# degleris1/CMF.jl

Measured on AMD Instinct MI355X. Metric: MU iters/sec (convolutive NMF multiplicative update; achieved HBM GB/s in `hbm`), higher is better.
Workload: dtype f32

## Files before the change

### cmf.jl_amd/csrc/cmf_api.hip

```cpp
#include "cmf_internal.h"

static void wb_free(cmf_handle_s *h);
static void wb_disarm(cmf_handle_s *h);

size_t n_partial(const cmf_handle_s *h)
{
    const CmfDims &d = h->d;
    size_t n = (size_t)(64 * h->conv_gx) * (size_t)std::max(h->conv_gy, h->conv_gy_ext);
    n = std::max(n, (size_t)(d.Np / 64) * d.KB * d.L);
    n = std::max(n, (size_t)((d.Tl + 63) / 64) * d.KB);
    n = std::max(n, 2 * (((size_t)d.Tl * d.K32 + 1023) / 1024));
    return n;
}

static int ensure_stage(cmf_handle_s *h, size_t elems)
{
    if (h->stage_elems >= elems) return CMF_OK;
    if (h->stage) HIPCHK(hipFree(h->stage));
    h->stage = nullptr;
    h->stage_elems = 0;
    HIPCHK(hipMalloc(&h->stage, elems * sizeof(double)));
    h->stage_elems = elems;
    return CMF_OK;
}
// ... 328 lines not shown
        for (const Want &w : wants) {
            *w.pp = static_cast<char *>(h->arena) + off;
            off += (w.bytes + 255) & ~(size_t)255;
        }
        h->numden = h->numden_own;
        for (int w = 0; w < 4; ++w) h->halo[w] = h->halo_own[w];
        h->d_scalar = h->d_scalar_own;
    }
    HIPB(hipHostMalloc(&h->h_scalar, 4 * sizeof(double)));
    if (data) {
        TRYB(upload_cols(h, data, 0, Tl, true, true));
        if (h->halo_r > 0) TRYB(upload_cols(h, data + (size_t)Tl * N, Tl, h->halo_r, false, false));
        h->data_norm = std::sqrt(h->data_sumsq);
        h->have_data = true;
    }
#undef TRYB
#undef HIPB
    *out = h;
    return CMF_OK;
}


int launch_hxt_on(cmf_handle_s *h, const float *X0, const float *X1, int NpX, int nsrc, float *slabs, int nchunks, int chunk_len,
                         int main_rows)
{
    ProfScope prof_(h, hxt_prof_class(h, X0, nsrc));
    const CmfDims &d = h->d;
    h->spec_gen = -1;
    HxtParams p;
    p.H = h->H; p.X0 = X0; p.X1 = X1; p.slabs = slabs;
    p.Np = NpX; p.K32 = d.K32; p.KB = d.KB; p.PADL = d.PADL; p.L = d.L; p.Tl = main_rows >= 0 ? main_rows : d.Tl; p.chunk_len = chunk_len;
    p.G = h->hxt_groups; p.nsrc = nsrc;
    p.CG = hxt_cg(nchunks);
    dim3 grid((NpX / 128) * p.CG * h->hxt_groups, nchunks / p.CG, nsrc * d.KB), block(256);
    switch (h->hxt_LP) {
#define CASE(LP_) case LP_: hipLaunchKernelGGL((hxt_kernel<LP_>), grid, block, 0, h->stream, p); break;
        CASE(1) CASE(2) CASE(3) CASE(4) CASE(5) CASE(6) CASE(8)
#undef CASE
    default: return fail(CMF_ERR_STATE, "internal: bad hxt LP %d", h->hxt_LP);
    }
    for (int i = 0; i < 7; ++i)
        if (kHxtLP[i] == h->hxt_LP) h->launches[LA_HXT + i] += 1;
    h->launches[nsrc == 1 ? LA_HXT_NSRC1 : LA_HXT_NSRC2] += 1;
    h->launches[p.Tl < d.Tl ? LA_HXT_TAIL : LA_HXT_NO_TAIL] += 1;
    KCHK("hxt_kernel");
    return CMF_OK;
}

int launch_transconv(cmf_handle_s *h, int nsrc, const float *xt0, bool front_block)
{
    if (h->sk_tc) return launch_transconv_small(h, nsrc, xt0);
    ProfScope prof_(h, nsrc == 2 ? PROF_TRANSCONV : PROF_TRANSCONV_1);
    const CmfDims &d = h->d;
    TcParams p;
    p.Wn = h->Wn; p.XT0 = xt0 ? xt0 : h->XT; p.XT1 = h->estT; p.slabs = h->hslabs;
    p.NpW = d.Np;
    p.TP = d.TP; p.PADL = d.PADL; p.K32 = d.K32; p.KB = d.KB; p.L = d.L; p.Tl = d.Tl;
    p.nsrc = nsrc;
    p.C = (int)(rup(d.N, 8) / 8);
    p.W = nsrc == 2 ? h->tc_W : h->tc_W1;
    p.F = nsrc == 2 ? h->tc_S : h->tc_S1;
    p.wtab = h->tc_tab[nsrc == 2 ? 0 : 1];
    p.t_first = 0;
    p.slab_rows = d.Tl;
    if (front_block) {
        p.W = h->tc_W2; p.F = h->tc_S2; p.wtab = h->tc_tab[2];
        p.t_first = -128;
        p.slab_rows = d.Tl + 128;
// ... 8 lines not shown
    h->launches[LA_TC + h->tc_LT / 4 - 1] += 1;
    if (front_block) h->launches[LA_TC_FRONT] += 1;
    if (p.W >= 64 && p.W % 32 == 0) h->launches[LA_TC_XCD] += 1;
    KCHK("transconv_kernel");
    return CMF_OK;
}

int launch_slab_sum(cmf_handle_s *h, float *out, const float *in, int nslabs, size_t stride, bool take_carry,
                           CmfHxtTail tail)
{
    size_t n4 = stride / 4;
    int blocks = (int)std::min<size_t>(2048, (n4 + 255) / 256);
    CmfLossCarry carry{};
    if (take_carry && h->carry.partial) {
        carry = h->carry;
        h->carry = CmfLossCarry{};
    }
    hipLaunchKernelGGL(slab_sum_kernel, dim3(blocks + (carry.partial ? 1 : 0)), dim3(256), 0, h->stream, out, in, nslabs, stride, n4, carry, tail);
    h->launches[carry.partial ? LA_SLAB_SUM_CARRY : LA_SLAB_SUM] += 1;
    KCHK("slab_sum_kernel");
    return CMF_OK;
}

int hxt_contract(cmf_handle_s *h, const float *X0, const float *X1, int nsrc, float *out, bool take_carry, bool slabs_only)
{
    const CmfDims &d = h->d;
    h->spec_gen = -1;
    if (h->small_k) return hxt_contract_small(h, X0, X1, nsrc, out, take_carry, slabs_only);
    const int nch = nsrc == 2 ? h->hxt_nchunks : h->hxt_nchunks1, clen = nsrc == 2 ? h->hxt_chunk_len : h->hxt_chunk_len1;
    const int main_rows = nsrc == 2 ? h->hxt_main : h->hxt_main1;
    CMFTRY(launch_hxt_on(h, X0, X1, d.Np, nsrc, h->wslabs, nch, clen, main_rows));
    const CmfHxtTail tail{h->H, X0, X1, d.Tl - main_rows, d.PADL + main_rows, d.L, d.K32, d.Np};
    return launch_slab_sum(h, out, h->wslabs, hxt_nslabs(nch), (size_t)nsrc * d.L * d.K32 * d.Np, take_carry, tail);
}

int read_scalar(cmf_handle_s *h, int slot, double *v)
{
    HIPCHK(hipMemcpyAsync(h->h_scalar + slot, h->d_scalar + slot, sizeof(double), hipMemcpyDeviceToHost, h->stream));
    HIPCHK(hipStreamSynchronize(h->stream));
    *v = h->h_scalar[slot];
    return CMF_OK;
}

static int check_ready(cmf_handle_s *h, bool need_data)
{
    if (!h) return fail(CMF_ERR_ARG, "handle is NULL");
    if (h->root_only) return fail(CMF_ERR_STATE, "this entry needs a single-GPU handle, not the front handle of a cmf_create_multi group");
    HIPCHK(hipSetDevice(h->device));
    if (!h->factors_set) return fail(CMF_ERR_STATE, "factors not set: call cmf_set_factors first");
    if (need_data && !h->have_data) return fail(CMF_ERR_STATE, "handle was created without data");
    return CMF_OK;
}

// ... 19 lines not shown
    default: return fail(CMF_ERR_STATE, "internal: the MU rule launches no conv mode %d", conv_mode(family, base));
    }
}

static int mu_conv(cmf_handle_s *h, int base, float *out, int T_store, int gy)
{
    const MuForm &f = mu_form(h);
    return mu_launch_conv(h, base >= CONV_BASE_LOSS ? f.loss_family : f.store_family, base, out, T_store, gy, mu_buf(h, f.conv_data[base]));
}

static bool mu_est_current(const cmf_handle_s *h) { return h->reuse_est && h->est_kind == mu_est_kind(h); }

static bool w_speculated(cmf_handle_s *h)
{
    const bool hit = mu_form(h).square_fusions && h->spec_gen >= 0 && h->spec_gen == h->est_gen && mu_est_current(h) && !h->carry.partial;
    h->spec_gen = -1;
    if (hit) h->spec_hits += 1;
    return hit;
}

static int mu_contract_c2(cmf_handle_s *h, bool slabs_only)
{
    const MuForm &f = mu_form(h);
    return hxt_contract(h, mu_buf(h, f.c2_src[0]), mu_buf(h, f.c2_src[1]), f.c2_nsrc, slabs_only ? nullptr : h->numden, !slabs_only, slabs_only);
}

static int mu_contract_w(cmf_handle_s *h, bool slabs_only)
{
    if (w_speculated(h)) return CMF_OK;
    if (!mu_est_current(h)) CMFTRY(mu_conv(h, CONV_BASE_STORE, h->est, h->d.Tl, h->conv_gy));
    set_est(h, mu_est_kind(h));
    return mu_contract_c2(h, slabs_only);
}

int w_partial_impl(cmf_handle_s *h) { return mu_contract_w(h, false); }

int w_partial_half_impl(cmf_handle_s *h, int den)
{
    const CmfDims &d = h->d;
    const size_t LKN = (size_t)d.L * d.K32 * d.Np;
    if (den) {
        if (!(h->reuse_est && h->est_kind == EST_CONV))
            CMFTRY(launch_conv<CONV_EST>(h, h->est, d.Tl, h->conv_gy));
        set_est(h, EST_CONV);
    }
    const float *src = den ? h->est : h->X;
    return hxt_contract(h, src, src, 1, h->numden + (den ? LKN : 0), den != 0);
}

int w_apply_impl(cmf_handle_s *h, double l1W, double l2W, const float *tail_src, float *tail_dst, int tail_n, const float *den)
{
    const CmfDims &d = h->d;
    dim3 grid(d.Np / 64, d.KB, d.L);
    if (!den) den = h->numden + (size_t)d.L * d.K32 * d.Np;
    const bool root = mu_form(h).sqrt_update;
    hipLaunchKernelGGL(root ? w_update_sqrt_kernel : w_update_kernel, grid, dim3(256), 0, h->stream, h->Wt, h->Wn, h->numden, den,
                       d.N, d.K, d.L, d.Np, d.K32, (float)l1W, (float)(2.0 * l2W), tail_src, tail_dst, tail_n);
    KCHK(root ? "w_update_sqrt_kernel" : "w_update_kernel");
    set_est(h, EST_NONE);
    return CMF_OK;
}

static int w_phase_impl(cmf_handle_s *h, double l1W, double l2W)
{
    const CmfDims &d = h->d;
    const MuForm &f = mu_form(h);
    if (!(h->small_k && f.square_fusions)) {
        CMFTRY(w_partial_impl(h));
        if (f.kl_den()) {
            hipLaunchKernelGGL(kl_hsum_kernel, dim3(d.K, KL_HCHUNKS), dim3(256), 0, h->stream, h->Ht, d.TP, d.PADL, d.Tl, h->kl_sums);
            KCHK("kl_hsum_kernel");
            hipLaunchKernelGGL(kl_den_w_kernel, dim3(d.L, d.K), dim3(256), 0, h->stream, h->Ht, h->kl_sums, h->numden + (size_t)d.L * d.K32 * d.Np, d.TP, d.PADL, d.Tl,
                               d.K32, d.Np);
            KCHK("kl_den_w_kernel");
        }
        return w_apply_impl(h, l1W, l2W);
    }
    CMFTRY(mu_contract_w(h, true));
    CmfLossCarry carry{};
    if (h->carry.partial) {
// ... 510 lines not shown
{
    if (!h) return fail(CMF_ERR_ARG, "handle is NULL");
    if (h->group) return group_sync(h->group);
    HIPCHK(hipSetDevice(h->device));
    HIPCHK(hipStreamSynchronize(h->stream));
    return CMF_OK;
}

int cmf_rccl_version(int *version, char *path, int64_t path_len)
{
    if (!version) return fail(CMF_ERR_ARG, "version is NULL");
    CMFTRY(rccl_load());
    RCCLCHK(g_rccl.GetVersion(version));
    if (path && path_len > 0) snprintf(path, (size_t)path_len, "%s", g_rccl.path.c_str());
    return CMF_OK;
}

int cmf_get_counter(cmf_handle h, const char *name, int64_t *value)
{
    if (!h || !name || !value) return fail(CMF_ERR_ARG, "NULL argument");
    if (std::strcmp(name, "hals_pipeline_reruns") == 0) { *value = h->hals_reruns; return CMF_OK; }
    if (std::strcmp(name, "writeback_calls") == 0) { *value = h->wb ? h->wb->armed_calls : 0; return CMF_OK; }
    if (std::strcmp(name, "speculated_contractions") == 0) { *value = h->spec_hits; return CMF_OK; }
    if (std::strcmp(name, "liveness_checks") == 0) { *value = g_liveness_checks.load(); return CMF_OK; }
    if (admm_counter(h, name, value)) return CMF_OK;
    if (sep_counter(h, name, value)) return CMF_OK;
    if (anls_counter(h, name, value)) return CMF_OK;
    if (std::strcmp(name, "small_k_fused_h_updates") == 0) {
        *value = h->sk_fused_h;
        if (h->group)
            for (const cmf_handle_s *s : h->group->sh) *value += (s != h) ? s->sk_fused_h : 0;
        return CMF_OK;
    }
    if (std::strcmp(name, "writeback_overlapped") == 0) { *value = h->wb ? h->wb->hooked_calls : 0; return CMF_OK; }
    if (std::strncmp(name, "launches:", 9) == 0) {
        for (int c = 0; c < LA_NCLS; ++c)
            if (std::strcmp(name + 9, kLaunchNames[c]) == 0) {
                *value = h->launches[c];
                if (h->group)
                    for (const cmf_handle_s *s : h->group->sh) *value += (s != h) ? s->launches[c] : 0;
                return CMF_OK;
            }
        return fail(CMF_ERR_ARG, "unknown launch path '%s'", name + 9);
    }
    if (h->group) {
        cmf_group_s *g = h->group;
// ... 39 lines not shown
    return CMF_OK;
}

int cmf_set_option(cmf_handle h, const char *name, int value)
{
    if (!h || !name) return fail(CMF_ERR_ARG, "NULL argument");
    if (std::strcmp(name, "anls_backup_only") == 0) {
        if (h->group || h->root_only || h->sharded) return fail(CMF_ERR_UNSUPPORTED, "anls_backup_only: the ANLS rule runs on single-GPU handles only");
        if (value != 0 && value != 1) return fail(CMF_ERR_ARG, "anls_backup_only must be 0 or 1");
        h->anls_backup_only = value;
        return CMF_OK;
    }
    if (std::strcmp(name, "nnls_large") == 0) {
        if (h->group || h->root_only || h->sharded) return fail(CMF_ERR_UNSUPPORTED, "nnls_large: the ANLS rule and the separable fit run on single-GPU handles only");
        if (value != 0 && value != 1) return fail(CMF_ERR_ARG, "nnls_large must be 0 or 1");
        h->nnls_large = value;
        return CMF_OK;
    }
    if (std::strcmp(name, "kl_mask") == 0) {
        if (h->group || h->root_only || h->sharded) return fail(CMF_ERR_UNSUPPORTED, "kl_mask: the mask and the divergence of the MU rule are chosen on single-GPU handles only");
        if (value != 0 && value != 1) return fail(CMF_ERR_ARG, "kl_mask must be 0 or 1");
        if (!value && h->mu_mask && h->mu_div) return fail(CMF_ERR_STATE, "kl_mask: the KL form and a mask are both installed; clear the mask or restore CMF_DIV_SQUARE first");
        h->kl_mask = value;
        return CMF_OK;
    }
    if (std::strcmp(name, "is_div") == 0) {
        if (h->group || h->root_only || h->sharded) return fail(CMF_ERR_UNSUPPORTED, "is_div: the divergence of the MU rule is chosen on single-GPU handles only");
        if (value != 0 && value != 1) return fail(CMF_ERR_ARG, "is_div must be 0 or 1");
        if (!value && h->mu_div == CMF_DIV_IS) return fail(CMF_ERR_STATE, "is_div: the Itakura-Saito divergence is installed; restore CMF_DIV_SQUARE with cmf_mu_set_divergence first");
        h->is_div = value;
        return CMF_OK;
    }
    if (h->group) {
        cmf_group_s *g = h->group;
        CMFTRY(group_join(g));
        if (std::strcmp(name, "allreduce_overlap") == 0) {
            CMFTRY(group_sync(g));
            if (value) CMFTRY(group_ensure_lane1(g));
            g->overlap = value != 0;
            g->num_ready = false;
            return CMF_OK;
        }
        if (std::strcmp(name, "halo_in_allreduce") == 0) {
            CMFTRY(group_sync(g));
            g->halo_opt = value != 0;
            g->halos_current = false;
// ... 1176 lines not shown
```

### cmf.jl_amd/csrc/cmf_internal.h

```cpp
#pragma once
#pragma GCC visibility push(default)
#include "cmf_hip.h"
#pragma GCC visibility pop
#include "cmf_kernels.h"
#include "cmf_rng.h"
#include "cmf_writeback.h"

#include <algorithm>
#include <atomic>
#include <chrono>
#include <cmath>
#include <cstdarg>
#include <cstdio>
#include <cstring>
#include <functional>
#include <map>
#include <mutex>
#include <string>
#include <thread>
#include <vector>

inline thread_local std::string g_err;

static int fail(int code, const char *fmt, ...)
// ... 232 lines not shown
    bool have_data = false;
    bool reuse_est = true;
    int gram = 0;
    float *gram_numden_h = nullptr;
    bool prof = false;
    int prof_every = 1;
    int prof_seen[32] = {0};
    int64_t launches[LA_NCLS] = {0};
    struct ProfRec { hipEvent_t a, b; int cls; };
    unsigned prof_mask = 0;
    std::vector<ProfRec> prof_recs;
    std::vector<hipEvent_t> prof_pool;
    int est_kind = EST_NONE;
    void *arena = nullptr;
    size_t arena_bytes = 0;
    bool streams_may_hang = false;
    int64_t est_gen = 0;
    int64_t spec_gen = -1;
    int last_rule_call = 0;
    bool speculate = true;
    std::function<int()> after_reduce;
    int64_t hals_spec_gen = -1;
    int64_t spec_hits = 0;

    struct cmf_group_s *group = nullptr;
    bool root_only = false;
    hipStream_t own_comm_stream = nullptr, comm_stream = nullptr;
    hipEvent_t ev_c0 = nullptr, ev_c1 = nullptr;
    double *h_ring = nullptr;
    bool dev_stamps = false;
    CmfLossCarry carry{};
    CmfWriteback *wb = nullptr;
    struct AdmmState *admm = nullptr;
    struct AnlsState *anls = nullptr;
    struct SepState *sep = nullptr;
    int anls_backup_only = 0;
    int nnls_large = 0;
};

void admm_free(cmf_handle_s *h);
int admm_counter(const cmf_handle_s *h, const char *name, int64_t *value);
void anls_free(cmf_handle_s *h);
int anls_counter(const cmf_handle_s *h, const char *name, int64_t *value);
void sep_free(cmf_handle_s *h);
int sep_counter(const cmf_handle_s *h, const char *name, int64_t *value);

// ... 146 lines not shown
int gram_w_impl(cmf_handle_s *h, double l1W, double l2W);
int gram_w_partial(cmf_handle_s *h, float *hh_out);
int gram_w_finish(cmf_handle_s *h, const float *HH, double l1W, double l2W, const float *tail_src = nullptr, float *tail_dst = nullptr,
                         int tail_n = 0);
int gram_h_update(cmf_handle_s *h, double l1H, double l2H);
int gram_h_impl(cmf_handle_s *h, double l1H, double l2H, double *loss);
int pgd_w_impl(cmf_handle_s *h, double pen_sq, double pen_abs, int nonneg);
int pgd_h_impl(cmf_handle_s *h, double pen_sq, double pen_abs, int nonneg, double *loss);
int hals_h_impl(cmf_handle_s *h, double l1H, double l2H);
int hals_h_rerun(cmf_handle_s *h);
int gram_denom_h(cmf_handle_s *h, float *out);
int gram_tables(cmf_handle_s *h);
int group_pgd_w(cmf_handle_s *st, struct cmf_group_s *g, double pen_sq, double pen_abs, int nonneg);
int group_pgd_h(cmf_handle_s *st, struct cmf_group_s *g, double pen_sq, double pen_abs, int nonneg, double *loss);
int group_set_mask(struct cmf_group_s *g, const double *mask);
size_t n_partial(const cmf_handle_s *h);
hipError_t stream_acquire(int device, hipStream_t *s);
void plan(cmf_handle_s *h, int n_cu);
int upload_cols(cmf_handle_s *h, const double *src, int64_t tc, int64_t ncols, bool rows_layout, bool accumulate_sumsq,
                       float *rows_dst = nullptr, float *cols_dst = nullptr);
int create_impl(cmf_handle *out, int device, int64_t N, int64_t Tl, int64_t K, int64_t L,
                       const double *data, int64_t t_offset, int64_t T_global, bool sharded);
int launch_hxt_on(cmf_handle_s *h, const float *X0, const float *X1, int NpX, int nsrc, float *slabs, int nchunks, int chunk_len,
                         int main_rows = -1);
int launch_transconv(cmf_handle_s *h, int nsrc, const float *xt0 = nullptr, bool front_block = false);
int launch_slab_sum(cmf_handle_s *h, float *out, const float *in, int nslabs, size_t stride, bool take_carry = false,
                           CmfHxtTail tail = CmfHxtTail{nullptr, nullptr, nullptr, 0, 0, 0, 0, 0});
int hxt_contract(cmf_handle_s *h, const float *X0, const float *X1, int nsrc, float *out, bool take_carry = false, bool slabs_only = false);
int hxt_contract_small(cmf_handle_s *h, const float *X0, const float *X1, int nsrc, float *out, bool take_carry, bool slabs_only);
bool sk_can_fuse_h(const cmf_handle_s *h);
int launch_transconv_small(cmf_handle_s *h, int nsrc, const float *xt0, bool update_h = false, float l1 = 0.f, float two_l2 = 0.f);
int read_scalar(cmf_handle_s *h, int slot, double *v);
int w_partial_impl(cmf_handle_s *h);
int w_partial_half_impl(cmf_handle_s *h, int den);
int w_apply_impl(cmf_handle_s *h, double l1W, double l2W, const float *tail_src = nullptr, float *tail_dst = nullptr, int tail_n = 0,
                        const float *den = nullptr);
int h_update_impl(cmf_handle_s *h, double l1H, double l2H, bool front = false);
int launch_loss_conv(cmf_handle_s *h);
int loss_partial_impl(cmf_handle_s *h, double *sumsq, bool readback = true, double *host_out = nullptr, bool speculate = false);
int set_factors_impl(cmf_handle_s *h, const double *W, const double *H);
int get_factors_impl(cmf_handle_s *h, double *W, double *H);
int reduce_partials(cmf_handle_s *h, const double *partial, int n, int slot, double *v);
double wait_timeout_s();
int ensure_resid(cmf_handle_s *h, bool masked = false, bool loss_abs = false);
HalsRowParams hals_row_params(cmf_handle_s *h, double l1H, double l2H);
int hals_persist_launch(cmf_handle_s *h, const HalsRowParams &q, int debug = 0, bool clear_flags = true);
int pgd_unit_norm(cmf_handle_s *h, bool is_W);
int rccl_load();
int group_use(cmf_handle_s *s);
int group_join(cmf_group_s *g);
int group_start_workers(cmf_group_s *g);
// ... 243 lines not shown
```

### cmf.jl_amd/csrc/cmf_kernels.h

```cpp
#pragma once
#include <hip/hip_runtime.h>
#include <type_traits>
#include <stdint.h>
#include "cmf_conv_modes.h"

typedef float f32x16 __attribute__((ext_vector_type(16)));
typedef float f32x4 __attribute__((ext_vector_type(4)));

#define CMF_EPS_F 2.220446049250313e-16f

struct CmfDims {
    int N, Tl, K, L;
    int Np;
    int KB;
    int K32;
    int PADL;
    int TP;
    int Lp;
};

__device__ __forceinline__ int cmf_crow(int r, int h) { return (r & 3) + 8 * (r >> 2) + 4 * h; }

__device__ __forceinline__ __amdgpu_buffer_rsrc_t cmf_rsrc(const void *base, size_t bytes)
{
// ... 1154 lines not shown
{
    __shared__ __attribute__((aligned(16))) float Hs[32 * CONV3_STRIDE];
    const int b = blockIdx.x;
    if (b < n_full) {
        const int n0 = (b % gx) * 64;
        if (n0 + 32 < p.N) conv3_tile<MODE, 2, NKP, PREQ>(p, Hs, (b / gx) * 64, n0, threadIdx.x, b);
        else conv3_tile<MODE, 1, NKP>(p, Hs, (b / gx) * 64, n0, threadIdx.x, b);
    } else {
        const int q = b - n_full, tile = n_full + (q >> 2), sub = q & 3;
        conv3_quarter<MODE, NKP>(p, Hs, (tile / gx) * 64 + (sub >> 1) * 32, (tile % gx) * 64 + (sub & 1) * 32, threadIdx.x, b);
    }
}

struct HxtParams {
    const float *H;
    const float *X0;
    const float *X1;
    float *slabs;
    int Np, K32, KB, PADL, L, Tl;
    int chunk_len;
    int G;
    int nsrc;
    int CG;
};

template <int LP>
__device__ __forceinline__ void hxt_load(float (&E)[LP], float (&O)[LP], float (&B)[LP], __amdgpu_buffer_rsrc_t hr,
                                         __amdgpu_buffer_rsrc_t xr, int hoff, int xoff, int row, int K32, int Np)
{
#pragma unroll
    for (int u = 0; u < LP; ++u) {
        E[u] = cmf_bload(hr, hoff, (row + 2 * u + 1) * K32 * 4);
        O[u] = cmf_bload(hr, hoff, (row + 2 * u) * K32 * 4);
        B[u] = cmf_bload(xr, xoff, (row + 2 * u) * Np * 4);
    }
}

template <int LP>
__device__ __forceinline__ void hxt_group(f32x16 (&acc)[2 * LP], const float (&Ep)[LP], const float (&Op)[LP],
                                          const float (&Ec)[LP], const float (&Oc)[LP], const float (&Bc)[LP])
{
#pragma unroll
    for (int u = 0; u < LP; ++u) {
#pragma unroll
        for (int m = 0; m < LP; ++m) {
            const float ae = (u - m >= 0) ? Ec[(u - m >= 0) ? (u - m) : 0] : Ep[(u - m >= 0) ? 0 : (u - m + LP)];
            const float ao = (u - m >= 0) ? Oc[(u - m >= 0) ? (u - m) : 0] : Op[(u - m >= 0) ? 0 : (u - m + LP)];
            acc[2 * m] = __builtin_amdgcn_mfma_f32_32x32x2f32(ae, Bc[u], acc[2 * m], 0, 0, 0);
            acc[2 * m + 1] = __builtin_amdgcn_mfma_f32_32x32x2f32(ao, Bc[u], acc[2 * m + 1], 0, 0, 0);
        }
    }
}

template <int LP>
__global__ __launch_bounds__(256, 1) void hxt_kernel(HxtParams p)
{
    const int lane = threadIdx.x & 63, wave = __builtin_amdgcn_readfirstlane(threadIdx.x >> 6);
    const int i = lane & 31, h = lane >> 5;
    int quad, lg;
    if ((gridDim.x / p.G) % 8 == 0) {
        lg = (blockIdx.x >> 3) % p.G;
        quad = (blockIdx.x & 7) + 8 * (blockIdx.x / (8 * p.G));
    } else {
        quad = blockIdx.x / p.G;
        lg = blockIdx.x % p.G;
    }
    const int CG = p.CG;
    const int cw = wave % CG, nw = wave / CG;
    const int nb = quad * (4 / CG) + nw;
    const int c = blockIdx.y * CG + cw;
    const int src = blockIdx.z % p.nsrc;
    const int kb = blockIdx.z / p.nsrc;
    const int lag0 = lg * 2 * LP;
    const int Np = p.Np, K32 = p.K32;
    const float *X = src ? p.X1 : p.X0;

    const int tc0 = c * p.chunk_len;
    int tc1 = tc0 + p.chunk_len;
    if (tc1 > p.Tl) tc1 = p.Tl;
    const int ngroups = (tc1 > tc0) ? (tc1 - tc0 + 6 * LP - 1) / (6 * LP) * 3 : 0;

    const float *hbase = p.H + (size_t)(p.PADL + tc0 - lag0 - 2 * LP - 1) * K32;
    const float *xbase = X + (size_t)(p.PADL + tc0 - 2 * LP) * Np;
    const __amdgpu_buffer_rsrc_t hr = cmf_rsrc(hbase, (size_t)(p.chunk_len + 12 * LP + 8) * K32 * 4);
    const __amdgpu_buffer_rsrc_t xr = cmf_rsrc(xbase, (size_t)(p.chunk_len + 12 * LP + 8) * Np * 4);
    const int hoff = (h * K32 + kb * 32 + i) * 4;
    const int xoff = (h * Np + nb * 32 + i) * 4;

    f32x16 acc[2 * LP];
#pragma unroll
    for (int a = 0; a < 2 * LP; ++a)
#pragma unroll
        for (int r = 0; r < 16; ++r) acc[a][r] = 0.f;

    float E0[LP], O0[LP], B0[LP], E1[LP], O1[LP], B1[LP], E2[LP], O2[LP], B2[LP];
    if (ngroups > 0) {
        hxt_load<LP>(E0, O0, B0, hr, xr, hoff, xoff, 0, K32, Np);
        hxt_load<LP>(E1, O1, B1, hr, xr, hoff, xoff, 2 * LP, K32, Np);
#define HXT_SCHED()                                                                   \
    do {                                                                              \
        constexpr int per = (2 * LP * LP >= 9 * LP) ? 2 : ((2 * LP * LP >= 6 * LP) ? 1 : 0);  \
        _Pragma("unroll") for (int q = 0; q < 3 * LP; ++q) {                          \
            __builtin_amdgcn_sched_group_barrier(0x020, 1, 0);                        \
            __builtin_amdgcn_sched_group_barrier(0x008, per, 0);                      \
        }                                                                             \
        __builtin_amdgcn_sched_group_barrier(0x008, 2 * LP * LP - per * 3 * LP, 0);   \
        __builtin_amdgcn_sched_barrier(0);                                            \
    } while (0)
        for (int g = 0; g < ngroups; g += 3) {
            const int g3 = (g + 3 < ngroups) ? g + 3 : g;
            hxt_load<LP>(E2, O2, B2, hr, xr, hoff, xoff, 2 * LP * (g + 2), K32, Np);
            hxt_group<LP>(acc, E0, O0, E1, O1, B1);
            HXT_SCHED();
            hxt_load<LP>(E0, O0, B0, hr, xr, hoff, xoff, 2 * LP * (g + 3), K32, Np);
            hxt_group<LP>(acc, E1, O1, E2, O2, B2);
            HXT_SCHED();
            hxt_load<LP>(E1, O1, B1, hr, xr, hoff, xoff, 2 * LP * (g3 + 1), K32, Np);
            hxt_group<LP>(acc, E2, O2, E0, O0, B0);
            HXT_SCHED();
        }
#undef HXT_SCHED
    }

    float *slab = p.slabs + (size_t)(blockIdx.y * p.nsrc + src) * p.L * K32 * Np;
    if (CG == 1) {
#pragma unroll
        for (int a = 0; a < 2 * LP; ++a) {
            int l = lag0 + a;
            if (l < p.L) {
#pragma unroll
                for (int r = 0; r < 16; ++r) {
                    int k = kb * 32 + cmf_crow(r, h);
                    slab[((size_t)l * K32 + k) * Np + nb * 32 + i] = acc[a][r];
                }
            }
        }
        return;
    }
    __shared__ float red[2][4][16][64];
#pragma unroll
    for (int a = 0; a < 2 * LP; ++a) {
        const int buf = a & 1;
#pragma unroll
        for (int r = 0; r < 16; ++r) red[buf][wave][r][lane] = acc[a][r];
        __syncthreads();
        const int l = lag0 + a;
        const int per = 16 / CG;
        for (int rr = 0; rr < per; ++rr) {
            const int r = cw * per + rr;
            float sum = red[buf][nw * CG][r][lane];
            for (int v = 1; v < CG; ++v) sum += red[buf][nw * CG + v][r][lane];
            const int k = kb * 32 + cmf_crow(r, h);
            if (l < p.L) slab[((size_t)l * K32 + k) * Np + nb * 32 + i] = sum;
        }
    }
}

struct TcParams {
    const float *Wn;
    const float *XT0;
    const float *XT1;
    float *slabs;
    int NpW;
    int TP, PADL, K32, KB, L, Tl;
    int nsrc;
    int C;
    int t_first;
    int slab_rows;
    int W;
    int F;
    const int4 *wtab;
};

#define TC_ROW 160
#define TC_CHUNK (8 * TC_ROW)

template <int LT>
// ... 140 lines not shown
        frag = 0;
    }
}

__device__ __forceinline__ float cmf_mu(float x, float num, float den, float l1, float two_l2)
{
    float d = ((den + l1) + two_l2 * x) + CMF_EPS_F;
    float y = x * (num / d);
    return (y != y) ? y : fmaxf(CMF_EPS_F, y);
}

__device__ __forceinline__ float cmf_mu_sqrt(float x, float num, float den, float l1, float two_l2)
{
    float d = ((den + l1) + two_l2 * x) + CMF_EPS_F;
    float y = x * sqrtf(num / d);
    return (y != y) ? y : fmaxf(CMF_EPS_F, y);
}
template <bool SQRT>
__device__ __forceinline__ float cmf_mu_step(float x, float num, float den, float l1, float two_l2)
{
    return SQRT ? cmf_mu_sqrt(x, num, den, l1, two_l2) : cmf_mu(x, num, den, l1, two_l2);
}

#define CMF_W_UPDATE_KERNEL(NAME, STEP)                                                                                                  \
    static __global__ __launch_bounds__(256) void NAME(float *Wt, float *Wn, const float *num_p, const float *den_p,                     \
                                                       int N, int K, int L, int Np, int K32, float l1, float two_l2,                     \
                                                       const float *tail_src, float *tail_dst, int tail_n)                               \
    {                                                                                                                                    \
        __shared__ float tile[32][65];                                                                                                   \
        const int tid = threadIdx.x;                                                                                                     \
        if (tail_dst && blockIdx.x == 0 && blockIdx.y == 0 && blockIdx.z == 0 && tid < tail_n)    \
            __hip_atomic_store(tail_dst + tid, tail_src[tid], __ATOMIC_RELAXED, __HIP_MEMORY_SCOPE_SYSTEM);  \
        const int n0 = blockIdx.x * 64, kb = blockIdx.y, l = blockIdx.z;                                                                 \
        {                                                                                                                                \
            const int nn = tid & 63;                                                                                                     \
            _Pragma("unroll") for (int q = 0; q < 8; ++q) {                                                                              \
                int kk = q * 4 + (tid >> 6);                                                                                             \
                int k = kb * 32 + kk, n = n0 + nn;                                                                                       \
                size_t idx = ((size_t)l * K32 + k) * Np + n;                                                                             \
                const float num = num_p[idx], den = den_p[idx];                                                                          \
                float w = Wt[idx];                                                                                                       \
                float wn = (k < K && n < N) ? STEP(w, num, den, l1, two_l2) : 0.f;                                                       \
                Wt[idx] = wn;                                                                                                            \
                tile[kk][nn] = wn;                                                                                                       \
            }                                                                                                                            \
        }                                                                                                                                \
        __syncthreads();                                                                                                                 \
        {                                                                                                                                \
            const int kk = tid & 31;                                                                                                     \
            _Pragma("unroll") for (int q = 0; q < 8; ++q) {                                                                              \
                int nn = q * 8 + (tid >> 5);                                                                                             \
                Wn[((size_t)l * Np + n0 + nn) * K32 + kb * 32 + kk] = tile[kk][nn];                                                      \
            }                                                                                                                            \
        }                                                                                                                                \
    }
CMF_W_UPDATE_KERNEL(w_update_kernel, cmf_mu)
// ... 54 lines not shown
            for (int c = 0; c < 4; ++c) hn[c] = (k + c < K) ? cmf_mu_step<SQRT>(x[c], num[c], den[c], l1, two_l2) : 0.f;
            *hp = hn;
        }
#pragma unroll
        for (int c = 0; c < 4; ++c) tile[4 * k4 + c][tt] = hn[c];
    }
    __syncthreads();
    {
        const int kk = tid >> 3, t2 = t0 + (tid & 7);
        if (t2 < Tl) Ht[(size_t)(kb * 32 + kk) * TP + PADL + t2] = tile[kk][tid & 7];
    }
}
static __global__ __launch_bounds__(256) void h_update_kernel(float *H, float *Ht, const float *nump, size_t num_stride, int Snum,
                                                        const float *denp, size_t den_stride, int Sden,
                                                        int Tl, int K, int K32, int PADL, int TP, float l1, float two_l2)
{
    h_update_body<false>(H, Ht, nump, num_stride, Snum, denp, den_stride, Sden, Tl, K, K32, PADL, TP, l1, two_l2);
}
static __global__ __launch_bounds__(256) void h_update_sqrt_kernel(float *H, float *Ht, const float *nump, size_t num_stride, int Snum,
                                                             const float *denp, size_t den_stride, int Sden,
                                                             int Tl, int K, int K32, int PADL, int TP, float l1, float two_l2)
{
    h_update_body<true>(H, Ht, nump, num_stride, Snum, denp, den_stride, Sden, Tl, K, K32, PADL, TP, l1, two_l2);
}

__device__ __forceinline__ double cmf_thread_loss_sum(const double *partial, int n)
{
    double s[8] = {0.0, 0.0, 0.0, 0.0, 0.0, 0.0, 0.0, 0.0};
    for (int base = threadIdx.x; base < n; base += 4 * 8 * 256) {
        double v[4][8];
#pragma unroll
        for (int q = 0; q < 4; ++q)
#pragma unroll
            for (int u = 0; u < 8; ++u) {
                const int e = base + 2048 * q + 256 * u;
                v[q][u] = partial[e < n ? e : 0];
            }
#pragma unroll
        for (int q = 0; q < 4; ++q)
#pragma unroll
            for (int u = 0; u < 8; ++u) s[u] += (base + 2048 * q + 256 * u < n) ? v[q][u] : 0.0;
    }
    return ((s[0] + s[1]) + (s[2] + s[3])) + ((s[4] + s[5]) + (s[6] + s[7]));
}

struct CmfLossCarry {
    const double *partial;
    int n;
    double *out;
    double *host_out;
    float *tail;
    int tail_len, rank;
};

__device__ __forceinline__ void cmf_block_loss_reduce(const CmfLossCarry &c)
{
    __shared__ double red[256];
    red[threadIdx.x] = cmf_thread_loss_sum(c.partial, c.n);
    __syncthreads();
    for (int off = 128; off > 0; off >>= 1) {
        if ((int)threadIdx.x < off) red[threadIdx.x] += red[threadIdx.x + off];
        __syncthreads();
    }
    const double tot = red[0];
    if (threadIdx.x == 0) {
        *c.out = tot;
        if (c.host_out) __hip_atomic_store(c.host_out, tot, __ATOMIC_RELAXED, __HIP_MEMORY_SCOPE_SYSTEM);
    }
    if (c.tail) {
        const float hi = (float)tot, lo = (float)(tot - (double)hi);
        for (int j = threadIdx.x; j < c.tail_len; j += 256) c.tail[j] = (j == 2 * c.rank) ? hi : (j == 2 * c.rank + 1) ? lo : 0.f;
    }
}

struct CmfHxtTail {
    const float *H, *X0, *X1;
    int rows, t0, L, K32, Np;
};

static __global__ __launch_bounds__(256) void slab_sum_kernel(float *out, const float *in, int nslabs, size_t stride, size_t n4, CmfLossCarry carry,
                                                        CmfHxtTail tail)
{
    unsigned bx = blockIdx.x, nbx = gridDim.x;
    if (carry.partial) {
        if (bx == 0) { cmf_block_loss_reduce(carry); return; }
        --bx; --nbx;
    }
    for (size_t idx = bx * (size_t)blockDim.x + threadIdx.x; idx < n4; idx += (size_t)nbx * blockDim.x) {
        float4 a = reinterpret_cast<const float4 *>(in)[idx];
        for (int s = 1; s < nslabs; s += 4) {
            float4 b[4];
#pragma unroll
            for (int u = 0; u < 4; ++u) {
                const int su = (s + u < nslabs) ? s + u : s;
                b[u] = reinterpret_cast<const float4 *>(in + (size_t)su * stride)[idx];
// ... 1877 lines not shown
```

Measured before the change: 187.7.

## Fuse H·Xᵀ chunk reduction and tail into an 8-wave direct kernel

Adds hxt_direct_kernel, which launches 512-thread blocks where each of 8 waves accumulates one time chunk. The partial sums are reduced in shared memory, the tail rows are added from LDS-staged X/H, and the result is written straight to numden. This removes the slab write, the separate slab_sum kernel and its intermediate HBM traffic for the W contraction. The pending loss-reduction carry moves into an extra block of the W update kernel, since slab_sum no longer runs. The cost is fewer blocks with more threads each and two syncthreads per lag, which may lower parallelism.

```diff
diff --git a/cmf.jl_amd/csrc/cmf_api.hip b/cmf.jl_amd/csrc/cmf_api.hip
--- a/cmf.jl_amd/csrc/cmf_api.hip
+++ b/cmf.jl_amd/csrc/cmf_api.hip
@@ -374,7 +374,7 @@
 
 
 int launch_hxt_on(cmf_handle_s *h, const float *X0, const float *X1, int NpX, int nsrc, float *slabs, int nchunks, int chunk_len,
-                         int main_rows)
+                         int main_rows, bool direct)
 {
     ProfScope prof_(h, hxt_prof_class(h, X0, nsrc));
     const CmfDims &d = h->d;
@@ -384,18 +384,30 @@
     p.Np = NpX; p.K32 = d.K32; p.KB = d.KB; p.PADL = d.PADL; p.L = d.L; p.Tl = main_rows >= 0 ? main_rows : d.Tl; p.chunk_len = chunk_len;
     p.G = h->hxt_groups; p.nsrc = nsrc;
     p.CG = hxt_cg(nchunks);
-    dim3 grid((NpX / 128) * p.CG * h->hxt_groups, nchunks / p.CG, nsrc * d.KB), block(256);
-    switch (h->hxt_LP) {
+    p.tail_rows = direct ? d.Tl - p.Tl : 0;
+    if (direct) {
+        if (nchunks != 8 || h->hxt_LP > 5) return fail(CMF_ERR_STATE, "internal: the 8-wave C2 form needs 8 chunks and LP <= 5 (%d, %d)", nchunks, h->hxt_LP);
+        dim3 grid((NpX / 32) * h->hxt_groups, 1, nsrc * d.KB), block(512);
+        switch (h->hxt_LP) {
+#define CASE(LP_) case LP_: hipLaunchKernelGGL((hxt_direct_kernel<LP_>), grid, block, 0, h->stream, p); break;
+            CASE(1) CASE(2) CASE(3) CASE(4) CASE(5)
+#undef CASE
+        }
+        h->hxt_direct_launches += 1;
+    } else {
+        dim3 grid((NpX / 128) * p.CG * h->hxt_groups, nchunks / p.CG, nsrc * d.KB), block(256);
+        switch (h->hxt_LP) {
 #define CASE(LP_) case LP_: hipLaunchKernelGGL((hxt_kernel<LP_>), grid, block, 0, h->stream, p); break;
-        CASE(1) CASE(2) CASE(3) CASE(4) CASE(5) CASE(6) CASE(8)
+            CASE(1) CASE(2) CASE(3) CASE(4) CASE(5) CASE(6) CASE(8)
 #undef CASE
-    default: return fail(CMF_ERR_STATE, "internal: bad hxt LP %d", h->hxt_LP);
+        default: return fail(CMF_ERR_STATE, "internal: bad hxt LP %d", h->hxt_LP);
+        }
     }
     for (int i = 0; i < 7; ++i)
         if (kHxtLP[i] == h->hxt_LP) h->launches[LA_HXT + i] += 1;
     h->launches[nsrc == 1 ? LA_HXT_NSRC1 : LA_HXT_NSRC2] += 1;
     h->launches[p.Tl < d.Tl ? LA_HXT_TAIL : LA_HXT_NO_TAIL] += 1;
-    KCHK("hxt_kernel");
+    KCHK(direct ? "hxt_direct_kernel" : "hxt_kernel");
     return CMF_OK;
 }
 
@@ -450,13 +462,14 @@
     return CMF_OK;
 }
 
-int hxt_contract(cmf_handle_s *h, const float *X0, const float *X1, int nsrc, float *out, bool take_carry, bool slabs_only)
+int hxt_contract(cmf_handle_s *h, const float *X0, const float *X1, int nsrc, float *out, bool take_carry, bool slabs_only, bool direct_ok)
 {
     const CmfDims &d = h->d;
     h->spec_gen = -1;
     if (h->small_k) return hxt_contract_small(h, X0, X1, nsrc, out, take_carry, slabs_only);
     const int nch = nsrc == 2 ? h->hxt_nchunks : h->hxt_nchunks1, clen = nsrc == 2 ? h->hxt_chunk_len : h->hxt_chunk_len1;
     const int main_rows = nsrc == 2 ? h->hxt_main : h->hxt_main1;
+    if (direct_ok && h->hxt_direct && !h->group && !h->sharded && nch == 8 && h->hxt_LP <= 5) return launch_hxt_on(h, X0, X1, d.Np, nsrc, out, nch, clen, main_rows, true);
     CMFTRY(launch_hxt_on(h, X0, X1, d.Np, nsrc, h->wslabs, nch, clen, main_rows));
     const CmfHxtTail tail{h->H, X0, X1, d.Tl - main_rows, d.PADL + main_rows, d.L, d.K32, d.Np};
     return launch_slab_sum(h, out, h->wslabs, hxt_nslabs(nch), (size_t)nsrc * d.L * d.K32 * d.Np, take_carry, tail);
@@ -522,7 +535,7 @@
 static int mu_contract_c2(cmf_handle_s *h, bool slabs_only)
 {
     const MuForm &f = mu_form(h);
-    return hxt_contract(h, mu_buf(h, f.c2_src[0]), mu_buf(h, f.c2_src[1]), f.c2_nsrc, slabs_only ? nullptr : h->numden, !slabs_only, slabs_only);
+    return hxt_contract(h, mu_buf(h, f.c2_src[0]), mu_buf(h, f.c2_src[1]), f.c2_nsrc, slabs_only ? nullptr : h->numden, !slabs_only, slabs_only, !slabs_only);
 }
 
 static int mu_contract_w(cmf_handle_s *h, bool slabs_only)
@@ -554,8 +567,14 @@
     dim3 grid(d.Np / 64, d.KB, d.L);
     if (!den) den = h->numden + (size_t)d.L * d.K32 * d.Np;
     const bool root = mu_form(h).sqrt_update;
+    CmfLossCarry carry{};
+    if (h->carry.partial && !h->group) {
+        carry = h->carry;
+        h->carry = CmfLossCarry{};
+        grid.x += 1;
+    }
     hipLaunchKernelGGL(root ? w_update_sqrt_kernel : w_update_kernel, grid, dim3(256), 0, h->stream, h->Wt, h->Wn, h->numden, den,
-                       d.N, d.K, d.L, d.Np, d.K32, (float)l1W, (float)(2.0 * l2W), tail_src, tail_dst, tail_n);
+                       d.N, d.K, d.L, d.Np, d.K32, (float)l1W, (float)(2.0 * l2W), tail_src, tail_dst, tail_n, carry);
     KCHK(root ? "w_update_sqrt_kernel" : "w_update_kernel");
     set_est(h, EST_NONE);
     return CMF_OK;
@@ -1112,6 +1131,7 @@
     if (std::strcmp(name, "hals_pipeline_reruns") == 0) { *value = h->hals_reruns; return CMF_OK; }
     if (std::strcmp(name, "writeback_calls") == 0) { *value = h->wb ? h->wb->armed_calls : 0; return CMF_OK; }
     if (std::strcmp(name, "speculated_contractions") == 0) { *value = h->spec_hits; return CMF_OK; }
+    if (std::strcmp(name, "hxt_direct_launches") == 0) { *value = h->hxt_direct_launches; return CMF_OK; }
     if (std::strcmp(name, "liveness_checks") == 0) { *value = g_liveness_checks.load(); return CMF_OK; }
     if (admm_counter(h, name, value)) return CMF_OK;
     if (sep_counter(h, name, value)) return CMF_OK;
@@ -1197,6 +1217,11 @@
         if (value != 0 && value != 1) return fail(CMF_ERR_ARG, "kl_mask must be 0 or 1");
         if (!value && h->mu_mask && h->mu_div) return fail(CMF_ERR_STATE, "kl_mask: the KL form and a mask are both installed; clear the mask or restore CMF_DIV_SQUARE first");
         h->kl_mask = value;
+        return CMF_OK;
+    }
+    if (std::strcmp(name, "hxt_direct") == 0) {
+        if (value != 0 && value != 1) return fail(CMF_ERR_ARG, "hxt_direct must be 0 or 1");
+        h->hxt_direct = value != 0;
         return CMF_OK;
     }
     if (std::strcmp(name, "is_div") == 0) {
diff --git a/cmf.jl_amd/csrc/cmf_internal.h b/cmf.jl_amd/csrc/cmf_internal.h
--- a/cmf.jl_amd/csrc/cmf_internal.h
+++ b/cmf.jl_amd/csrc/cmf_internal.h
@@ -278,6 +278,8 @@
     std::function<int()> after_reduce;
     int64_t hals_spec_gen = -1;
     int64_t spec_hits = 0;
+    bool hxt_direct = true;
+    int64_t hxt_direct_launches = 0;
 
     struct cmf_group_s *group = nullptr;
     bool root_only = false;
@@ -470,11 +472,12 @@
 int create_impl(cmf_handle *out, int device, int64_t N, int64_t Tl, int64_t K, int64_t L,
                        const double *data, int64_t t_offset, int64_t T_global, bool sharded);
 int launch_hxt_on(cmf_handle_s *h, const float *X0, const float *X1, int NpX, int nsrc, float *slabs, int nchunks, int chunk_len,
-                         int main_rows = -1);
+                         int main_rows = -1, bool direct = false);
 int launch_transconv(cmf_handle_s *h, int nsrc, const float *xt0 = nullptr, bool front_block = false);
 int launch_slab_sum(cmf_handle_s *h, float *out, const float *in, int nslabs, size_t stride, bool take_carry = false,
                            CmfHxtTail tail = CmfHxtTail{nullptr, nullptr, nullptr, 0, 0, 0, 0, 0});
-int hxt_contract(cmf_handle_s *h, const float *X0, const float *X1, int nsrc, float *out, bool take_carry = false, bool slabs_only = false);
+int hxt_contract(cmf_handle_s *h, const float *X0, const float *X1, int nsrc, float *out, bool take_carry = false, bool slabs_only = false,
+                 bool direct_ok = false);
 int hxt_contract_small(cmf_handle_s *h, const float *X0, const float *X1, int nsrc, float *out, bool take_carry, bool slabs_only);
 bool sk_can_fuse_h(const cmf_handle_s *h);
 int launch_transconv_small(cmf_handle_s *h, int nsrc, const float *xt0, bool update_h = false, float l1 = 0.f, float two_l2 = 0.f);
diff --git a/cmf.jl_amd/csrc/cmf_kernels.h b/cmf.jl_amd/csrc/cmf_kernels.h
--- a/cmf.jl_amd/csrc/cmf_kernels.h
+++ b/cmf.jl_amd/csrc/cmf_kernels.h
@@ -1200,6 +1200,7 @@
     int G;
     int nsrc;
     int CG;
+    int tail_rows;
 };
 
 template <int LP>
@@ -1231,28 +1232,9 @@
 }
 
 template <int LP>
-__global__ __launch_bounds__(256, 1) void hxt_kernel(HxtParams p)
-{
-    const int lane = threadIdx.x & 63, wave = __builtin_amdgcn_readfirstlane(threadIdx.x >> 6);
-    const int i = lane & 31, h = lane >> 5;
-    int quad, lg;
-    if ((gridDim.x / p.G) % 8 == 0) {
-        lg = (blockIdx.x >> 3) % p.G;
-        quad = (blockIdx.x & 7) + 8 * (blockIdx.x / (8 * p.G));
-    } else {
-        quad = blockIdx.x / p.G;
-        lg = blockIdx.x % p.G;
-    }
-    const int CG = p.CG;
-    const int cw = wave % CG, nw = wave / CG;
-    const int nb = quad * (4 / CG) + nw;
-    const int c = blockIdx.y * CG + cw;
-    const int src = blockIdx.z % p.nsrc;
-    const int kb = blockIdx.z / p.nsrc;
-    const int lag0 = lg * 2 * LP;
+__device__ __forceinline__ void hxt_accumulate(const HxtParams &p, const float *X, int nb, int kb, int lag0, int c, int i, int h, f32x16 (&acc)[2 * LP])
+{
     const int Np = p.Np, K32 = p.K32;
-    const float *X = src ? p.X1 : p.X0;
-
     const int tc0 = c * p.chunk_len;
     int tc1 = tc0 + p.chunk_len;
     if (tc1 > p.Tl) tc1 = p.Tl;
@@ -1265,7 +1247,6 @@
     const int hoff = (h * K32 + kb * 32 + i) * 4;
     const int xoff = (h * Np + nb * 32 + i) * 4;
 
-    f32x16 acc[2 * LP];
 #pragma unroll
     for (int a = 0; a < 2 * LP; ++a)
 #pragma unroll
@@ -1299,6 +1280,33 @@
         }
 #undef HXT_SCHED
     }
+}
+
+template <int LP>
+__global__ __launch_bounds__(256, 1) void hxt_kernel(HxtParams p)
+{
+    const int lane = threadIdx.x & 63, wave = __builtin_amdgcn_readfirstlane(threadIdx.x >> 6);
+    const int i = lane & 31, h = lane >> 5;
+    int quad, lg;
+    if ((gridDim.x / p.G) % 8 == 0) {
+        lg = (blockIdx.x >> 3) % p.G;
+        quad = (blockIdx.x & 7) + 8 * (blockIdx.x / (8 * p.G));
+    } else {
+        quad = blockIdx.x / p.G;
+        lg = blockIdx.x % p.G;
+    }
+    const int CG = p.CG;
+    const int cw = wave % CG, nw = wave / CG;
+    const int nb = quad * (4 / CG) + nw;
+    const int c = blockIdx.y * CG + cw;
+    const int src = blockIdx.z % p.nsrc;
+    const int kb = blockIdx.z / p.nsrc;
+    const int lag0 = lg * 2 * LP;
+    const int Np = p.Np, K32 = p.K32;
+    const float *X = src ? p.X1 : p.X0;
+
+    f32x16 acc[2 * LP];
+    hxt_accumulate<LP>(p, X, nb, kb, lag0, c, i, h, acc);
 
     float *slab = p.slabs + (size_t)(blockIdx.y * p.nsrc + src) * p.L * K32 * Np;
     if (CG == 1) {
@@ -1331,6 +1339,78 @@
             const int k = kb * 32 + cmf_crow(r, h);
             if (l < p.L) slab[((size_t)l * K32 + k) * Np + nb * 32 + i] = sum;
         }
+    }
+}
+
+template <int LP>
+__global__ __launch_bounds__(512, 1) void hxt_direct_kernel(HxtParams p)
+{
+    __shared__ float red[8][16][64];
+    __shared__ __attribute__((aligned(16))) float tailX[6 * LP][32];
+    __shared__ __attribute__((aligned(16))) float tailH[8 * LP][32];
+    const int lane = threadIdx.x & 63, wave = __builtin_amdgcn_readfirstlane(threadIdx.x >> 6);
+    const int i = lane & 31, h = lane >> 5;
+    int nb, lg;
+    if ((gridDim.x / p.G) % 8 == 0) {
+        lg = (blockIdx.x >> 3) % p.G;
+        nb = (blockIdx.x & 7) + 8 * (blockIdx.x / (8 * p.G));
+    } else {
+        nb = blockIdx.x / p.G;
+        lg = blockIdx.x % p.G;
+    }
+    const int src = blockIdx.z % p.nsrc;
+    const int kb = blockIdx.z / p.nsrc;
+    const int lag0 = lg * 2 * LP;
+    const int Np = p.Np, K32 = p.K32;
+    const float *X = src ? p.X1 : p.X0;
+
+    const int trows = p.tail_rows, t0 = p.PADL + p.Tl;
+    if (trows > 0) {
+        for (int e = threadIdx.x; e < trows * 32; e += 512) tailX[e >> 5][e & 31] = X[(size_t)(t0 + (e >> 5)) * Np + nb * 32 + (e & 31)];
+        for (int e = threadIdx.x; e < (trows + 2 * LP - 1) * 32; e += 512)
+            tailH[e >> 5][e & 31] = p.H[(size_t)(t0 - lag0 - (2 * LP - 1) + (e >> 5)) * K32 + kb * 32 + (e & 31)];
+    }
+
+    f32x16 acc[2 * LP];
+    hxt_accumulate<LP>(p, X, nb, kb, lag0, wave, i, h, acc);
+
+    const int r0 = 2 * wave, k0 = cmf_crow(r0, h);
+    float *out = p.slabs + (size_t)src * p.L * K32 * Np;
+#pragma unroll
+    for (int a = 0; a < 2 * LP; ++a) {
+#pragma unroll
+        for (int r = 0; r < 16; ++r) red[wave][r][lane] = acc[a][r];
+        __syncthreads();
+        float sum[2];
+#pragma unroll
+        for (int rr = 0; rr < 2; ++rr) {
+            float first = red[0][r0 + rr][lane], second = red[4][r0 + rr][lane];
+#pragma unroll
+            for (int v = 1; v < 4; ++v) {
+                first += red[v][r0 + rr][lane];
+                second += red[4 + v][r0 + rr][lane];
+            }
+            sum[rr] = first + second;
+        }
+        const int l = lag0 + a;
+        if (l < p.L) {
+            for (int u0 = 0; u0 < trows; u0 += 2 * LP) {
+                float xv[2 * LP];
+                float2 hv[2 * LP];
+#pragma unroll
+                for (int u = 0; u < 2 * LP; ++u) {
+                    const int uu = (u0 + u < trows) ? u0 + u : u0;
+                    xv[u] = tailX[uu][i];
+                    hv[u] = *reinterpret_cast<const float2 *>(&tailH[uu - a + 2 * LP - 1][k0]);
+                }
+#pragma unroll
+                for (int u = 0; u < 2 * LP; ++u)
+                    if (u0 + u < trows) { sum[0] = fmaf(hv[u].x, xv[u], sum[0]); sum[1] = fmaf(hv[u].y, xv[u], sum[1]); }
+            }
+#pragma unroll
+            for (int rr = 0; rr < 2; ++rr) out[((size_t)l * K32 + kb * 32 + k0 + rr) * Np + nb * 32 + i] = sum[rr];
+        }
+        __syncthreads();
     }
 }
 
@@ -1517,16 +1597,73 @@
     return SQRT ? cmf_mu_sqrt(x, num, den, l1, two_l2) : cmf_mu(x, num, den, l1, two_l2);
 }
 
+__device__ __forceinline__ double cmf_thread_loss_sum(const double *partial, int n)
+{
+    double s[8] = {0.0, 0.0, 0.0, 0.0, 0.0, 0.0, 0.0, 0.0};
+    for (int base = threadIdx.x; base < n; base += 4 * 8 * 256) {
+        double v[4][8];
+#pragma unroll
+        for (int q = 0; q < 4; ++q)
+#pragma unroll
+            for (int u = 0; u < 8; ++u) {
+                const int e = base + 2048 * q + 256 * u;
+                v[q][u] = partial[e < n ? e : 0];
+            }
+#pragma unroll
+        for (int q = 0; q < 4; ++q)
+#pragma unroll
+            for (int u = 0; u < 8; ++u) s[u] += (base + 2048 * q + 256 * u < n) ? v[q][u] : 0.0;
+    }
+    return ((s[0] + s[1]) + (s[2] + s[3])) + ((s[4] + s[5]) + (s[6] + s[7]));
+}
+
+struct CmfLossCarry {
+    const double *partial;
+    int n;
+    double *out;
+    double *host_out;
+    float *tail;
+    int tail_len, rank;
+};
+
+__device__ __forceinline__ void cmf_block_loss_reduce(const CmfLossCarry &c)
+{
+    __shared__ double red[256];
+    red[threadIdx.x] = cmf_thread_loss_sum(c.partial, c.n);
+    __syncthreads();
+    for (int off = 128; off > 0; off >>= 1) {
+        if ((int)threadIdx.x < off) red[threadIdx.x] += red[threadIdx.x + off];
+        __syncthreads();
+    }
+    const double tot = red[0];
+    if (threadIdx.x == 0) {
+        *c.out = tot;
+        if (c.host_out) __hip_atomic_store(c.host_out, tot, __ATOMIC_RELAXED, __HIP_MEMORY_SCOPE_SYSTEM);
+    }
+    if (c.tail) {
+        const float hi = (float)tot, lo = (float)(tot - (double)hi);
+        for (int j = threadIdx.x; j < c.tail_len; j += 256) c.tail[j] = (j == 2 * c.rank) ? hi : (j == 2 * c.rank + 1) ? lo : 0.f;
+    }
+}
+
 #define CMF_W_UPDATE_KERNEL(NAME, STEP)                                                                                                  \
     static __global__ __launch_bounds__(256) void NAME(float *Wt, float *Wn, const float *num_p, const float *den_p,                     \
                                                        int N, int K, int L, int Np, int K32, float l1, float two_l2,                     \
-                                                       const float *tail_src, float *tail_dst, int tail_n)                               \
+                                                       const float *tail_src, float *tail_dst, int tail_n, CmfLossCarry carry)           \
     {                                                                                                                                    \
         __shared__ float tile[32][65];                                                                                                   \
         const int tid = threadIdx.x;                                                                                                     \
         if (tail_dst && blockIdx.x == 0 && blockIdx.y == 0 && blockIdx.z == 0 && tid < tail_n)    \
             __hip_atomic_store(tail_dst + tid, tail_src[tid], __ATOMIC_RELAXED, __HIP_MEMORY_SCOPE_SYSTEM);  \
-        const int n0 = blockIdx.x * 64, kb = blockIdx.y, l = blockIdx.z;                                                                 \
+        unsigned bx = blockIdx.x;                                                                                                        \
+        if (carry.partial) {        \
+            if (bx == 0) {                                                                                                               \
+                if (blockIdx.y == 0 && blockIdx.z == 0) cmf_block_loss_reduce(carry);                                                    \
+                return;                                                                                                                  \
+            }                                                                                                                            \
+            --bx;                                                                                                                        \
+        }                                                                                                                                \
+        const int n0 = bx * 64, kb = blockIdx.y, l = blockIdx.z;                                                                         \
         {                                                                                                                                \
             const int nn = tid & 63;                                                                                                     \
             _Pragma("unroll") for (int q = 0; q < 8; ++q) {                                                                              \
@@ -1627,55 +1764,6 @@
                                                              int Tl, int K, int K32, int PADL, int TP, float l1, float two_l2)
 {
     h_update_body<true>(H, Ht, nump, num_stride, Snum, denp, den_stride, Sden, Tl, K, K32, PADL, TP, l1, two_l2);
-}
-
-__device__ __forceinline__ double cmf_thread_loss_sum(const double *partial, int n)
-{
-    double s[8] = {0.0, 0.0, 0.0, 0.0, 0.0, 0.0, 0.0, 0.0};
-    for (int base = threadIdx.x; base < n; base += 4 * 8 * 256) {
-        double v[4][8];
-#pragma unroll
-        for (int q = 0; q < 4; ++q)
-#pragma unroll
-            for (int u = 0; u < 8; ++u) {
-                const int e = base + 2048 * q + 256 * u;
-                v[q][u] = partial[e < n ? e : 0];
-            }
-#pragma unroll
-        for (int q = 0; q < 4; ++q)
-#pragma unroll
-            for (int u = 0; u < 8; ++u) s[u] += (base + 2048 * q + 256 * u < n) ? v[q][u] : 0.0;
-    }
-    return ((s[0] + s[1]) + (s[2] + s[3])) + ((s[4] + s[5]) + (s[6] + s[7]));
-}
-
-struct CmfLossCarry {
-    const double *partial;
-    int n;
-    double *out;
-    double *host_out;
-    float *tail;
-    int tail_len, rank;
-};
-
-__device__ __forceinline__ void cmf_block_loss_reduce(const CmfLossCarry &c)
-{
-    __shared__ double red[256];
-    red[threadIdx.x] = cmf_thread_loss_sum(c.partial, c.n);
-    __syncthreads();
-    for (int off = 128; off > 0; off >>= 1) {
-        if ((int)threadIdx.x < off) red[threadIdx.x] += red[threadIdx.x + off];
-        __syncthreads();
-    }
-    const double tot = red[0];
-    if (threadIdx.x == 0) {
-        *c.out = tot;
-        if (c.host_out) __hip_atomic_store(c.host_out, tot, __ATOMIC_RELAXED, __HIP_MEMORY_SCOPE_SYSTEM);
-    }
-    if (c.tail) {
-        const float hi = (float)tot, lo = (float)(tot - (double)hi);
-        for (int j = threadIdx.x; j < c.tail_len; j += 256) c.tail[j] = (j == 2 * c.rank) ? hi : (j == 2 * c.rank + 1) ? lo : 0.f;
-    }
 }
 
 struct CmfHxtTail {
```

Result: no change. 188.6, median of 6 (+0.5%).
